# zhoujoey/ORB-SLAM3-Mac

Hardware: AMD Instinct MI355X
Metric: ORB extract+match frames/sec (higher is better)
Workload: dtype u8; 1 GPU; vga: synthetic 640x480 batch=1024 per GPU, 8-level pyramid, 1000 feats/frame, ORB extract + Hamming 2-NN match (Frame.cc:1146) + SearchForInitialization (ORBmatcher.cc:710) vs successor frame; pipelines=1, matchers=side by side (two contexts), frames_total=1024

## Files before the change

### orb-slam3-mac_amd/csrc/match_kernels.hip

```cpp
#include "orb_internal.h"
#include "wave_dpp.h"
#include <climits>
#include <cstring>
#include <string>

struct orbhip_ctx;
hipStream_t orbhip_ctx_stream_internal(orbhip_ctx *c);
void orbhip_set_last_error_internal(const char *msg);
int orbhip_ctx_device_internal(orbhip_ctx *c);
int32_t *orbhip_ctx_status_internal(orbhip_ctx *c);

extern "C" int orbhip_descriptor_distance(const uint8_t *a32, const uint8_t *b32)
{
    int dist = 0;
    for (int i = 0; i < 8; i++) {
        uint32_t pa, pb;
        memcpy(&pa, a32 + 4 * i, 4); memcpy(&pb, b32 + 4 * i, 4);
        uint32_t v = pa ^ pb;
        v = v - ((v >> 1) & 0x55555555);
        v = (v & 0x33333333) + ((v >> 2) & 0x33333333);
        dist += (((v + (v >> 4)) & 0xF0F0F0F) * 0x1010101) >> 24;
    }
    return dist;
}

__device__ __forceinline__ int hamming256(const uint4 &a0, const uint4 &a1, const uint4 &b0, const uint4 &b1)
{
    return __popc(a0.x ^ b0.x) + __popc(a0.y ^ b0.y) + __popc(a0.z ^ b0.z) + __popc(a0.w ^ b0.w) +
           __popc(a1.x ^ b1.x) + __popc(a1.y ^ b1.y) + __popc(a1.z ^ b1.z) + __popc(a1.w ^ b1.w);
}

__device__ __forceinline__ int wave_incl_scan_i(int v) { return wave_scan_add_dpp(v); }

#define BF_TILE 256
__device__ __forceinline__ bool bf_slice(const int32_t *nA, const int32_t *nB, const int32_t *monoA, const int32_t *monoB, int pair, int max_n,
                                         int &na, int &nb, int &ma, int &mb)
{
    na = nA[pair]; nb = nB[pair]; ma = 0; mb = 0;
    if (!monoA) return true;
    if (na > max_n || nb > max_n) return false;
    ma = min(max(monoA[pair], 0), max(na, 0)); mb = min(max(monoB[pair], 0), max(nb, 0));
    na -= ma; nb -= mb;
    return true;
}
template <bool MONO>
__global__ __launch_bounds__(256) void k_bf2nn(const uint8_t *descA, const int32_t *nA, size_t strideA,
                                               const uint8_t *descB, const int32_t *nB, size_t strideB,
                                               int max_n, double ratio, int32_t *idx2, int32_t *dist2, uint8_t *accept,
                                               const int32_t *monoA, const int32_t *monoB)
{
    __shared__ uint4 tile[BF_TILE * 2];
    const int pair = blockIdx.y, tid = threadIdx.x;
    int na, nb, ma, mb;
    if (!bf_slice(nA, nB, MONO ? monoA : nullptr, monoB, pair, max_n, na, nb, ma, mb)) return;
    const int q = blockIdx.x * 256 + tid;
    if (blockIdx.x * 256 >= na) return;
    const uint4 *A = reinterpret_cast<const uint4 *>(descA + (size_t)pair * strideA) + 2 * (size_t)ma;
    const uint4 *B = reinterpret_cast<const uint4 *>(descB + (size_t)pair * strideB) + 2 * (size_t)mb;
    uint4 a0 = make_uint4(0, 0, 0, 0), a1 = a0;
    if (q < na) { a0 = A[2 * q]; a1 = A[2 * q + 1]; }
    uint32_t kb = 0xFFFFFFFFu, ks = 0xFFFFFFFFu;
    for (int t0 = 0; t0 < nb; t0 += BF_TILE) {
        const int tn = min(BF_TILE, nb - t0);
        __syncthreads();
        for (int i = tid; i < tn * 2; i += 256) tile[i] = B[2 * t0 + i];
        __syncthreads();
#pragma unroll 4
        for (int j = 0; j < tn; j++) {
            const uint32_t key = ((uint32_t)hamming256(a0, a1, tile[2 * j], tile[2 * j + 1]) << 16) | (uint32_t)(t0 + j);
            ks = min(ks, max(kb, key));
            kb = min(kb, key);
        }
    }
    if (q < na) {
        const int best = kb == 0xFFFFFFFFu ? INT_MAX : (int)(kb >> 16), second = ks == 0xFFFFFFFFu ? INT_MAX : (int)(ks >> 16);
        const int bi = kb == 0xFFFFFFFFu ? -1 : (int)(kb & 0xFFFFu), si = ks == 0xFFFFFFFFu ? -1 : (int)(ks & 0xFFFFu);
        const size_t o = ((size_t)pair * max_n + q) * 2;
        idx2[o] = bi; idx2[o + 1] = si; dist2[o] = best; dist2[o + 1] = second;
        accept[(size_t)pair * max_n + q] = (si >= 0 && (double)(float)best < (double)(float)second * ratio) ? 1 : 0;
    }
}

#define BFM_ROWB 272
typedef int bfm_v4i __attribute__((ext_vector_type(4)));
typedef int bfm_v16i __attribute__((ext_vector_type(16)));
__device__ __forceinline__ uint32_t bfm_widen4(uint32_t nib) { return __umul24(nib, 0x00204081u) & 0x01010101u; }
__device__ __forceinline__ uint32_t bfm_widen4_pm(uint32_t nib)
{
    uint32_t v = 0;
#pragma unroll
    for (int k = 0; k < 4; k++) v |= (((nib >> k) & 1u) ? 0xFFu : 0x01u) << (8 * k);
    return v;
}
#define BFM_WAVES 8
template <bool MONO>
__global__ __launch_bounds__(64 * BFM_WAVES) void k_bf2nn_mfma(const uint8_t *descA, const int32_t *nA, size_t strideA,
                                                    const uint8_t *descB, const int32_t *nB, size_t strideB,
                                                    int max_n, double ratio, int32_t *idx2, int32_t *dist2, uint8_t *accept,
                                                    const int32_t *monoA, const int32_t *monoB)
{
    __shared__ __attribute__((aligned(16))) uint8_t Bx[2 * 64 * BFM_ROWB];
    static_assert(BFM_WAVES * 2 * 8 * 64 * 4 <= 2 * 64 * BFM_ROWB, "the merge area (half of the rows at a time) fits the tile buffers");
    const int pair = blockIdx.y, tid = threadIdx.x, lane = tid & 63, wave = tid >> 6;
    int na, nb, ma, mb;
    if (!bf_slice(nA, nB, MONO ? monoA : nullptr, monoB, pair, max_n, na, nb, ma, mb)) return;
    const int q0 = blockIdx.x * (32 * BFM_WAVES);
    if (q0 >= na) return;
    const uint32_t *A = reinterpret_cast<const uint32_t *>(descA + (size_t)pair * strideA) + 8 * (size_t)ma;
    const uint32_t *B = reinterpret_cast<const uint32_t *>(descB + (size_t)pair * strideB) + 8 * (size_t)mb;
    const int r = lane & 31, h = lane >> 5;
    const int qrow = q0 + 32 * wave + r;
    bfm_v4i af[8];
    int pa_row = 0;
    {
        uint32_t w[8];
#pragma unroll
        for (int m = 0; m < 8; m++) { w[m] = qrow < na ? A[(size_t)8 * qrow + m] : 0u; pa_row += __popc(w[m]); }
#pragma unroll
        for (int m = 0; m < 8; m++) {
            const uint32_t hw = (w[m] >> (16 * h)) & 0xFFFFu;
            af[m] = (bfm_v4i){(int)bfm_widen4_pm(hw & 15u), (int)bfm_widen4_pm((hw >> 4) & 15u), (int)bfm_widen4_pm((hw >> 8) & 15u), (int)bfm_widen4_pm(hw >> 12)};
        }
    }
    bfm_v16i cinit;
#pragma unroll
    for (int g = 0; g < 16; g++) cinit[g] = __shfl(pa_row, (g & 3) + 8 * (g >> 2) + 4 * h, 64);
    uint32_t k1[16], k2[16];
#pragma unroll
    for (int g = 0; g < 16; g++) { k1[g] = 0xFFFFFFFFu; k2[g] = 0xFFFFFFFFu; }
    const int sc = tid >> 3, sm = tid & 7;
    auto fetch = [&](int t0, uint32_t &w0) { w0 = (t0 + sc < nb) ? B[(size_t)8 * (t0 + sc) + sm] : 0u; };
    auto widen = [&](int bufi, uint32_t w) {
        uint4 lo = make_uint4(bfm_widen4(w & 15u), bfm_widen4((w >> 4) & 15u), bfm_widen4((w >> 8) & 15u), bfm_widen4((w >> 12) & 15u));
        uint4 hi = make_uint4(bfm_widen4((w >> 16) & 15u), bfm_widen4((w >> 20) & 15u), bfm_widen4((w >> 24) & 15u), bfm_widen4(w >> 28));
        uint4 *dst = reinterpret_cast<uint4 *>(&Bx[bufi * 64 * BFM_ROWB + sc * BFM_ROWB + sm * 32]);
        dst[0] = lo; dst[1] = hi;
    };
    uint32_t nw0;
    fetch(0, nw0);
    widen(0, nw0);
    __syncthreads();
    int buf = 0;
    for (int t0 = 0; t0 < nb; t0 += 64, buf ^= 1) {
        const bool more = t0 + 64 < nb;
        if (more) fetch(t0 + 64, nw0);
#pragma unroll
        for (int half = 0; half < 2; half++) {
            if (t0 + 32 * half >= nb) break;
            bfm_v16i acc = cinit;
#pragma unroll
            for (int m = 0; m < 8; m++) {
                const bfm_v4i bf = *reinterpret_cast<const bfm_v4i *>(&Bx[buf * 64 * BFM_ROWB + (r + 32 * half) * BFM_ROWB + m * 32 + h * 16]);
                acc = __builtin_amdgcn_mfma_i32_32x32x32_i8(af[m], bf, acc, 0, 0, 0);
            }
            const int col = t0 + 32 * half + r;
            const uint32_t base = col < nb ? (uint32_t)col : (0x40000000u | (uint32_t)col);
#pragma unroll
            for (int g = 0; g < 16; g++) {
                const uint32_t key = ((uint32_t)acc[g] << 16) + base;
                asm("v_med3_u32 %0, %1, %2, %3" : "=v"(k2[g]) : "v"(k1[g]), "v"(key), "v"(k2[g]));
                k1[g] = min(k1[g], key);
            }
        }
        if (more) widen(buf ^ 1, nw0);
        __syncthreads();
    }
    uint32_t (*kout)[2][8][64] = reinterpret_cast<uint32_t (*)[2][8][64]>(&Bx[0]);
#pragma unroll
    for (int part = 0; part < 2; part++) {
        if (part) __syncthreads();
#pragma unroll
        for (int g = 0; g < 8; g++) { kout[wave][0][g][lane] = k1[8 * part + g]; kout[wave][1][g][lane] = k2[8 * part + g]; }
        __syncthreads();
        if (lane < 16) {
            const int row = 16 * part + lane, g = (row & 3) + 4 * ((row >> 3) & 1), hh = (row >> 2) & 1;
            uint32_t kb = 0xFFFFFFFFu, ks = 0xFFFFFFFFu;
            for (int c = 0; c < 32; c++) {
                const uint32_t a1 = kout[wave][0][g][32 * hh + c], a2 = kout[wave][1][g][32 * hh + c];
                ks = min(min(ks, a2), max(kb, a1));
                kb = min(kb, a1);
            }
            const int q = q0 + 32 * wave + row;
            if (q < na) {
                const bool hb = (kb >> 16) <= 256u, hs = (ks >> 16) <= 256u;
                const int best = hb ? (int)(kb >> 16) : INT_MAX, second = hs ? (int)(ks >> 16) : INT_MAX;
                const int bi = hb ? (int)(kb & 0xFFFFu) : -1, si = hs ? (int)(ks & 0xFFFFu) : -1;
                const size_t o = ((size_t)pair * max_n + q) * 2;
                idx2[o] = bi; idx2[o + 1] = si; dist2[o] = best; dist2[o + 1] = second;
                accept[(size_t)pair * max_n + q] = (si >= 0 && (double)(float)best < (double)(float)second * ratio) ? 1 : 0;
            }
        }
    }
}

extern "C" int orbhip_match_bf2nn_device(orbhip_ctx *ctx, const uint8_t *d_descA, const int32_t *d_nA, size_t strideA,
                                         const uint8_t *d_descB, const int32_t *d_nB, size_t strideB, int pairs,
                                         int max_n, double ratio, int32_t *d_idx2, int32_t *d_dist2, uint8_t *d_accept)
{
    if (!ctx || !d_descA || !d_descB || !d_nA || !d_nB || pairs <= 0 || max_n <= 0 || max_n > 65535 || !d_idx2 || !d_dist2 || !d_accept)
        return ORBHIP_E_BADARG;
    if (hipSetDevice(orbhip_ctx_device_internal(ctx)) != hipSuccess) return ORBHIP_E_HIP;
    if (max_n >= 64 && !getenv("ORBHIP_BF2NN_VALU")) {
        dim3 grid((max_n + 32 * BFM_WAVES - 1) / (32 * BFM_WAVES), pairs);
        hipLaunchKernelGGL(k_bf2nn_mfma<false>, grid, dim3(64 * BFM_WAVES), 0, orbhip_ctx_stream_internal(ctx), d_descA, d_nA, strideA, d_descB, d_nB,
                           strideB, max_n, ratio, d_idx2, d_dist2, d_accept, nullptr, nullptr);
    } else {
        dim3 grid((max_n + 255) / 256, pairs);
        hipLaunchKernelGGL(k_bf2nn<false>, grid, dim3(256), 0, orbhip_ctx_stream_internal(ctx), d_descA, d_nA, strideA, d_descB, d_nB,
                           strideB, max_n, ratio, d_idx2, d_dist2, d_accept, nullptr, nullptr);
    }
    return hipGetLastError() == hipSuccess ? ORBHIP_OK : ORBHIP_E_HIP;
}

int orbhip_bf2nn_slices_internal(orbhip_ctx *ctx, const uint8_t *d_descA, const int32_t *d_nA, const int32_t *d_monoA, size_t strideA,
                                 const uint8_t *d_descB, const int32_t *d_nB, const int32_t *d_monoB, size_t strideB, int pairs, int max_n,
                                 double ratio, int32_t *d_idx2, int32_t *d_dist2, uint8_t *d_accept)
{
    if (max_n >= 64 && !getenv("ORBHIP_BF2NN_VALU")) {
        dim3 grid((max_n + 32 * BFM_WAVES - 1) / (32 * BFM_WAVES), pairs);
        hipLaunchKernelGGL(k_bf2nn_mfma<true>, grid, dim3(64 * BFM_WAVES), 0, orbhip_ctx_stream_internal(ctx), d_descA, d_nA, strideA, d_descB, d_nB,
                           strideB, max_n, ratio, d_idx2, d_dist2, d_accept, d_monoA, d_monoB);
    } else {
        dim3 grid((max_n + 255) / 256, pairs);
        hipLaunchKernelGGL(k_bf2nn<true>, grid, dim3(256), 0, orbhip_ctx_stream_internal(ctx), d_descA, d_nA, strideA, d_descB, d_nB,
                           strideB, max_n, ratio, d_idx2, d_dist2, d_accept, d_monoA, d_monoB);
    }
    return hipGetLastError() == hipSuccess ? ORBHIP_OK : ORBHIP_E_HIP;
}

#define SI_COLS 64
#define SI_ROWS 48
#define SI_MAXN 8192
#define SI_CAP0 4096
#define SI_RANKS 2048
#define SI_TH_LOW 50
#define SI_HISTO 30

template <int NS>
__device__ __forceinline__ int si_register_loop(int lane, int n0, int na0, const float *kx, const float *ky, const uint16_t *cellx, const uint16_t *celly,
                                                const uint16_t *cpos, const uint16_t *gidx, const uint16_t *aidx, uint16_t *bm,
                                                const uint4 *dA, const uint4 *dB, const float *prev, int32_t *m12,
                                                float min_x, float min_y, float inv_w, float inv_h, float r, float nn_ratio)
{
    int nmatches = 0;
    float fkx[NS], fky[NS]; uint32_t fpk[NS]; int fgi[NS], fmd[NS], fm21[NS]; uint4 fd0[NS], fd1[NS];
#pragma unroll
    for (int sl = 0; sl < NS; sl++) {
        const int li = sl * 64 + lane;
        const bool v = li < n0;
        const int lj = v ? li : 0;
        fkx[sl] = kx[lj]; fky[sl] = ky[lj];
        fpk[sl] = v ? ((uint32_t)cellx[lj] | ((uint32_t)celly[lj] << 8) | ((uint32_t)min((int)cpos[lj], SI_RANKS - 1) << 16)) : 0xFFFFu;
        fgi[sl] = v ? (int)gidx[lj] : 0; fmd[sl] = INT_MAX; fm21[sl] = -1;
        fd0[sl] = dB[2 * fgi[sl]]; fd1[sl] = dB[2 * fgi[sl] + 1];
    }
    int qi[NS]; float qx[NS], qy[NS]; uint4 qd0[NS], qd1[NS];
#pragma unroll
    for (int sl = 0; sl < NS; sl++) {
        const int tq = sl * 64 + lane;
        qi[sl] = tq < na0 ? (int)aidx[tq] : 0;
        qx[sl] = prev[2 * qi[sl]]; qy[sl] = prev[2 * qi[sl] + 1];
        qd0[sl] = dA[2 * qi[sl]]; qd1[sl] = dA[2 * qi[sl] + 1];
    }
    for (int t = 0; t < na0; t++) {
        const int tsl = t >> 6, tln = t & 63;
        int i1 = 0; float x = 0, y = 0; uint4 a0 = make_uint4(0, 0, 0, 0), a1 = a0;
#define SI_RL(v) (uint32_t)__builtin_amdgcn_readlane((int)(v), tln)
#pragma unroll
        for (int sl = 0; sl < NS; sl++)
            if (tsl == sl) {
                i1 = (int)SI_RL(qi[sl]); x = __uint_as_float(SI_RL(__float_as_uint(qx[sl]))); y = __uint_as_float(SI_RL(__float_as_uint(qy[sl])));
                a0 = make_uint4(SI_RL(qd0[sl].x), SI_RL(qd0[sl].y), SI_RL(qd0[sl].z), SI_RL(qd0[sl].w));
                a1 = make_uint4(SI_RL(qd1[sl].x), SI_RL(qd1[sl].y), SI_RL(qd1[sl].z), SI_RL(qd1[sl].w));
            }
#undef SI_RL
        int c0 = (int)floorf(__fmul_rn(__fsub_rn(__fsub_rn(x, min_x), r), inv_w)); if (c0 < 0) c0 = 0;
        if (c0 >= SI_COLS) continue;
        int c1 = (int)ceilf(__fmul_rn(__fadd_rn(__fsub_rn(x, min_x), r), inv_w)); if (c1 > SI_COLS - 1) c1 = SI_COLS - 1;
        if (c1 < 0) continue;
        int r0 = (int)floorf(__fmul_rn(__fsub_rn(__fsub_rn(y, min_y), r), inv_h)); if (r0 < 0) r0 = 0;
        if (r0 >= SI_ROWS) continue;
        int r1 = (int)ceilf(__fmul_rn(__fadd_rn(__fsub_rn(y, min_y), r), inv_h)); if (r1 > SI_ROWS - 1) r1 = SI_ROWS - 1;
        if (r1 < 0) continue;
        const int ncy = r1 - r0 + 1;
        uint32_t lk1 = 0xFFFFFFFFu, ld2 = 0xFFFFFFFFu; int best_sl = 0;
        const uint32_t cw = (uint32_t)(c1 - c0), rh = (uint32_t)(r1 - r0);
#pragma unroll
        for (int sl = 0; sl < NS; sl++) {
            if (sl * 64 >= n0) break;
            const uint32_t dcx = (fpk[sl] & 255u) - (uint32_t)c0, dcy = ((fpk[sl] >> 8) & 255u) - (uint32_t)r0;
            const int dist = hamming256(a0, a1, fd0[sl], fd1[sl]);
            const bool c = dcx <= cw && dcy <= rh && fabsf(__fsub_rn(fkx[sl], x)) < r && fabsf(__fsub_rn(fky[sl], y)) < r && !(fmd[sl] <= dist);
            const uint32_t key = c ? ((uint32_t)dist << 23) | ((dcx * (uint32_t)ncy + dcy) * SI_RANKS + (fpk[sl] >> 16)) : 0xFFFFFFFFu;
            ld2 = min(ld2, max(lk1, key));
            best_sl = key < lk1 ? sl : best_sl;
            lk1 = min(lk1, key);
        }
        const uint32_t k1 = wave_min_u32_dpp(lk1);
        const uint32_t k2 = wave_min_u32_dpp(lk1 == k1 ? ld2 : lk1);
        const int d2 = k2 == 0xFFFFFFFFu ? INT_MAX : (int)(k2 >> 23);
        if (k1 == 0xFFFFFFFFu) continue;
        const int best = (int)(k1 >> 23);
        if (!(best <= SI_TH_LOW && (float)best < __fmul_rn((float)d2, nn_ratio))) continue;
        const unsigned long long owner = __ballot(lk1 == k1);
        const int ol = __builtin_amdgcn_readfirstlane(__ffsll((long long)owner) - 1);
        const int bsl = __builtin_amdgcn_readlane(best_sl, ol);
        int old = -1, best_idx = 0;
#pragma unroll
        for (int sl = 0; sl < NS; sl++)
            if (bsl == sl) {
                old = __builtin_amdgcn_readlane(fm21[sl], ol); best_idx = __builtin_amdgcn_readlane(fgi[sl], ol);
                if (lane == ol) { fm21[sl] = i1; fmd[sl] = best; }
            }
        if (old >= 0) nmatches--;
        nmatches++;
        if (lane == 0) {
            if (old >= 0) m12[old] = -1;
            m12[i1] = best_idx;
            bm[i1] = (uint16_t)best_idx;
        }
    }
    return nmatches;
}

__device__ __forceinline__ int si_tail(int lane, int n1, const orbhip_keypoint *kpA, const orbhip_keypoint *kpB, const uint16_t *bm, int8_t *bin_of,
                                       int *hist, int *s_keep, int32_t *m12, float *prev, int nmatches, int check_ori)
{
    const float factor = 1.0f / SI_HISTO;
    __syncthreads();
    if (check_ori) {
        for (int i1 = lane; i1 < n1; i1 += 64) {
            const int b = bm[i1];
            if (b == 0xFFFF) continue;
            float rot = __fsub_rn(kpA[i1].angle, kpB[b].angle);
            if (rot < 0.0f) rot = __fadd_rn(rot, 360.0f);
            int bin = (int)roundf(__fmul_rn(rot, factor));
            if (bin == SI_HISTO) bin = 0;
            atomicAdd(&hist[bin], 1); bin_of[i1] = (int8_t)bin;
        }
        __syncthreads();
        if (lane == 0) {
            int max1 = 0, max2 = 0, max3 = 0, ind1 = -1, ind2 = -1, ind3 = -1;
            for (int i = 0; i < SI_HISTO; i++) {
                const int sz = hist[i];
                if (sz > max1) { max3 = max2; max2 = max1; max1 = sz; ind3 = ind2; ind2 = ind1; ind1 = i; }
                else if (sz > max2) { max3 = max2; max2 = sz; ind3 = ind2; ind2 = i; }
                else if (sz > max3) { max3 = sz; ind3 = i; }
            }
            if ((float)max2 < __fmul_rn(0.1f, (float)max1)) { ind2 = -1; ind3 = -1; }
            else if ((float)max3 < __fmul_rn(0.1f, (float)max1)) ind3 = -1;
            s_keep[0] = ind1; s_keep[1] = ind2; s_keep[2] = ind3;
        }
        __syncthreads();
        int removed = 0;
        for (int i1 = lane; i1 < n1; i1 += 64) {
            const int b = bin_of[i1];
            if (b < 0 || b == s_keep[0] || b == s_keep[1] || b == s_keep[2]) continue;
            if (m12[i1] >= 0) { m12[i1] = -1; removed++; }
        }
        removed = wave_sum_dpp(removed);
        nmatches -= removed;
    }
    __syncthreads();
    for (int i1 = lane; i1 < n1; i1 += 64)
        if (m12[i1] >= 0) { prev[2 * i1] = kpB[m12[i1]].x; prev[2 * i1 + 1] = kpB[m12[i1]].y; }
    return nmatches;
}

#ifdef SI_PROF
__device__ long long g_si_prof[8];
#define SI_T(i) do { if (blockIdx.x == 0 && threadIdx.x == 0) { const long long t_ = clock64(); g_si_prof[i] += t_ - t_prev; t_prev = t_; } } while (0)
extern "C" int orbhip_debug_si_prof(long long *out8, int reset)
{
    if (out8 && hipMemcpyFromSymbol(out8, HIP_SYMBOL(g_si_prof), 64) != hipSuccess) return ORBHIP_E_HIP;
    if (reset) { long long z[8] = {0}; if (hipMemcpyToSymbol(HIP_SYMBOL(g_si_prof), z, 64) != hipSuccess) return ORBHIP_E_HIP; }
    return ORBHIP_OK;
}
#else
#define SI_T(i) do { } while (0)
#endif
__global__ __launch_bounds__(64) void k_search_init(const orbhip_keypoint *kpA_, const uint8_t *descA_, const int32_t *nA,
                                                    const orbhip_keypoint *kpB_, const uint8_t *descB_, const int32_t *nB,
                                                    int max_n, size_t kp_stride, float min_x, float min_y, float max_x, float max_y,
                                                    int window, float nn_ratio, int check_ori, int cap0, int maxn,
                                                    float *prev_, int32_t *m12_, int32_t *nmatches_, int32_t *status, const int32_t *redo_,
                                                    int32_t *redo_out)
{
    if (redo_ && !redo_[blockIdx.x]) { if (redo_out && threadIdx.x == 0) redo_out[blockIdx.x] = 0; return; }
    extern __shared__ __attribute__((aligned(16))) uint8_t si_lds[];
    float *kx = reinterpret_cast<float *>(si_lds), *ky = kx + cap0;
    int *matched_dist = reinterpret_cast<int *>(ky + cap0);
    uint32_t *cand_key = reinterpret_cast<uint32_t *>(matched_dist + cap0);
    uint16_t *cellx = reinterpret_cast<uint16_t *>(cand_key + cap0), *celly = cellx + cap0, *cpos = celly + cap0, *gidx = cpos + cap0;
    int16_t *m21 = reinterpret_cast<int16_t *>(gidx + cap0);
    uint16_t *aidx = reinterpret_cast<uint16_t *>(m21 + cap0), *cand_li = aidx + cap0;
    uint16_t *bm = cand_li + cap0;
    int8_t *bin_of = reinterpret_cast<int8_t *>(bm + maxn);
    __shared__ int hist[SI_HISTO];
    __shared__ int s_keep[3];
    const int pair = blockIdx.x, lane = threadIdx.x;
#ifdef SI_PROF
    long long t_prev = clock64();
#endif
    const unsigned long long lt_mask = (1ull << lane) - 1;
    const int n1 = nA[pair], n2 = nB[pair];
    const orbhip_keypoint *kpA = kpA_ + (size_t)pair * kp_stride, *kpB = kpB_ + (size_t)pair * kp_stride;
    const uint4 *dA = reinterpret_cast<const uint4 *>(descA_ + (size_t)pair * kp_stride * 32);
    const uint4 *dB = reinterpret_cast<const uint4 *>(descB_ + (size_t)pair * kp_stride * 32);
    float *prev = prev_ + (size_t)pair * max_n * 2;
    int32_t *m12 = m12_ + (size_t)pair * max_n;
    if (n1 > maxn || n2 > maxn) { if (lane == 0) { atomicExch(status, ORBHIP_E_CAPACITY); nmatches_[pair] = 0; } return; }
    const float inv_w = __fdiv_rn((float)SI_COLS, __fsub_rn(max_x, min_x));
    const float inv_h = __fdiv_rn((float)SI_ROWS, __fsub_rn(max_y, min_y));
    for (int i = lane; i < SI_HISTO; i += 64) hist[i] = 0;
    int n0 = 0;
    for (int i0 = 0; i0 < n2; i0 += 64) {
        const int i = i0 + lane;
        bool in = false; int px = 0, py = 0; float fx = 0, fy = 0;
        if (i < n2) {
            const orbhip_keypoint k = kpB[i];
            fx = k.x; fy = k.y;
            px = (int)roundf(__fmul_rn(__fsub_rn(fx, min_x), inv_w));
            py = (int)roundf(__fmul_rn(__fsub_rn(fy, min_y), inv_h));
            in = k.octave == 0 && px >= 0 && px < SI_COLS && py >= 0 && py < SI_ROWS;
        }
        const unsigned long long bal = __ballot(in);
        const int li = n0 + __popcll(bal & lt_mask);
        if (in && li < cap0) {
            kx[li] = fx; ky[li] = fy; cellx[li] = (uint16_t)px; celly[li] = (uint16_t)py; gidx[li] = (uint16_t)i;
            matched_dist[li] = INT_MAX; m21[li] = -1;
        }
        n0 += __popcll(bal);
    }
    int na0 = 0;
    for (int i0 = 0; i0 < n1; i0 += 64) {
        const int i = i0 + lane;
        const bool in = i < n1 && kpA[i].octave == 0;
        const unsigned long long bal = __ballot(in);
        const int li = na0 + __popcll(bal & lt_mask);
        if (in && li < cap0) aidx[li] = (uint16_t)i;
        na0 += __popcll(bal);
        if (i < n1) { m12[i] = -1; bin_of[i] = -1; bm[i] = 0xFFFFu; }
    }
    if (redo_out) {
        if (lane == 0) redo_out[pair] = (n0 > cap0 || na0 > cap0) ? 1 : 0;
        if (n0 > cap0 || na0 > cap0) return;
    }
    if (n0 > cap0 || na0 > cap0) { if (lane == 0) { atomicExch(status, ORBHIP_E_CAPACITY); nmatches_[pair] = 0; } return; }
    __syncthreads();
    for (int li = lane; li < n0; li += 64) {
        const int cx = cellx[li], cy = celly[li];
        int rank = 0;
        for (int j = 0; j < li; j++) rank += (cellx[j] == cx && celly[j] == cy);
        cpos[li] = (uint16_t)rank;
    }
    __syncthreads();
    SI_T(0);
    int nmatches = 0;
    const float r = (float)window;
    if (n0 <= 4 * 64 && na0 <= 4 * 64)
        nmatches = si_register_loop<4>(lane, n0, na0, kx, ky, cellx, celly, cpos, gidx, aidx, bm, dA, dB, prev, m12, min_x, min_y, inv_w, inv_h, r, nn_ratio);
    else if (n0 <= 8 * 64 && na0 <= 8 * 64)
        nmatches = si_register_loop<8>(lane, n0, na0, kx, ky, cellx, celly, cpos, gidx, aidx, bm, dA, dB, prev, m12, min_x, min_y, inv_w, inv_h, r, nn_ratio);
    else {
    int i1n = na0 > 0 ? (int)aidx[0] : 0;
    float xn = 0, yn = 0; uint4 pd0 = make_uint4(0, 0, 0, 0), pd1 = pd0;
    if (na0 > 0) { xn = prev[2 * i1n]; yn = prev[2 * i1n + 1]; pd0 = dA[2 * i1n]; pd1 = dA[2 * i1n + 1]; }
    for (int t = 0; t < na0; t++) {
        const int i1 = i1n;
        const float x = xn, y = yn;
        const uint4 a0 = pd0, a1 = pd1;
        if (t + 1 < na0) { i1n = aidx[t + 1]; xn = prev[2 * i1n]; yn = prev[2 * i1n + 1]; pd0 = dA[2 * i1n]; pd1 = dA[2 * i1n + 1]; }
        int c0 = (int)floorf(__fmul_rn(__fsub_rn(__fsub_rn(x, min_x), r), inv_w)); if (c0 < 0) c0 = 0;
        if (c0 >= SI_COLS) continue;
        int c1 = (int)ceilf(__fmul_rn(__fadd_rn(__fsub_rn(x, min_x), r), inv_w)); if (c1 > SI_COLS - 1) c1 = SI_COLS - 1;
        if (c1 < 0) continue;
        int r0 = (int)floorf(__fmul_rn(__fsub_rn(__fsub_rn(y, min_y), r), inv_h)); if (r0 < 0) r0 = 0;
        if (r0 >= SI_ROWS) continue;
        int r1 = (int)ceilf(__fmul_rn(__fadd_rn(__fsub_rn(y, min_y), r), inv_h)); if (r1 > SI_ROWS - 1) r1 = SI_ROWS - 1;
        if (r1 < 0) continue;
        const int ncy = r1 - r0 + 1;
        int ncand = 0;
        for (int l0 = 0; l0 < n0; l0 += 64) {
            const int li = l0 + lane;
            bool c = false; uint32_t key = 0;
            if (li < n0) {
                const int cx = cellx[li], cy = celly[li];
                c = cx >= c0 && cx <= c1 && cy >= r0 && cy <= r1 &&
                    fabsf(__fsub_rn(kx[li], x)) < r && fabsf(__fsub_rn(ky[li], y)) < r;
                key = (uint32_t)(((cx - c0) * ncy + (cy - r0)) * SI_RANKS + min((int)cpos[li], SI_RANKS - 1));
            }
            const unsigned long long bal = __ballot(c);
            if (c) { const int o = ncand + __popcll(bal & lt_mask); cand_li[o] = (uint16_t)li; cand_key[o] = key; }
// ... 1852 lines not shown
```

Before: 317,000 frames/s.

## Software-pipeline MFMA brute-force matcher, interleaving key retirement with next half-tile

Restructures the MFMA Hamming 2-NN loop so the top-2 key updates for one 32-column half-tile are interleaved with the MFMAs of the next half. The accumulator now starts at zero, with the per-row popcount bias applied only once at the end instead of shuffled into an initial accumulator. It also makes the ±1 nibble widening cheaper, adds an occupancy hint to launch_bounds, and spreads the final merge across four lanes per row with xor shuffles instead of serial 32-step loops on 16 lanes. The aim is to hide MFMA latency and cut VALU and merge overhead, at the cost of more complex tail handling and register pressure limits from the occupancy hint.

```diff
diff --git a/orb-slam3-mac_amd/csrc/match_kernels.hip b/orb-slam3-mac_amd/csrc/match_kernels.hip
--- a/orb-slam3-mac_amd/csrc/match_kernels.hip
+++ b/orb-slam3-mac_amd/csrc/match_kernels.hip
@@ -3,6 +3,7 @@
 #include <climits>
 #include <cstring>
 #include <string>
+#include <type_traits>
 
 struct orbhip_ctx;
 hipStream_t orbhip_ctx_stream_internal(orbhip_ctx *c);
@@ -87,14 +88,12 @@
 __device__ __forceinline__ uint32_t bfm_widen4(uint32_t nib) { return __umul24(nib, 0x00204081u) & 0x01010101u; }
 __device__ __forceinline__ uint32_t bfm_widen4_pm(uint32_t nib)
 {
-    uint32_t v = 0;
-#pragma unroll
-    for (int k = 0; k < 4; k++) v |= (((nib >> k) & 1u) ? 0xFFu : 0x01u) << (8 * k);
-    return v;
+    const uint32_t s = bfm_widen4(nib);
+    return ((s << 8) - s) | 0x01010101u;
 }
 #define BFM_WAVES 8
 template <bool MONO>
-__global__ __launch_bounds__(64 * BFM_WAVES) void k_bf2nn_mfma(const uint8_t *descA, const int32_t *nA, size_t strideA,
+__global__ __launch_bounds__(64 * BFM_WAVES, 4) void k_bf2nn_mfma(const uint8_t *descA, const int32_t *nA, size_t strideA,
                                                     const uint8_t *descB, const int32_t *nB, size_t strideB,
                                                     int max_n, double ratio, int32_t *idx2, int32_t *dist2, uint8_t *accept,
                                                     const int32_t *monoA, const int32_t *monoB)
@@ -121,15 +120,13 @@
             const uint32_t hw = (w[m] >> (16 * h)) & 0xFFFFu;
             af[m] = (bfm_v4i){(int)bfm_widen4_pm(hw & 15u), (int)bfm_widen4_pm((hw >> 4) & 15u), (int)bfm_widen4_pm((hw >> 8) & 15u), (int)bfm_widen4_pm(hw >> 12)};
         }
-    }
-    bfm_v16i cinit;
-#pragma unroll
-    for (int g = 0; g < 16; g++) cinit[g] = __shfl(pa_row, (g & 3) + 8 * (g >> 2) + 4 * h, 64);
+        asm volatile("" : "+v"(pa_row));
+    }
     uint32_t k1[16], k2[16];
 #pragma unroll
     for (int g = 0; g < 16; g++) { k1[g] = 0xFFFFFFFFu; k2[g] = 0xFFFFFFFFu; }
     const int sc = tid >> 3, sm = tid & 7;
-    auto fetch = [&](int t0, uint32_t &w0) { w0 = (t0 + sc < nb) ? B[(size_t)8 * (t0 + sc) + sm] : 0u; };
+    auto fetch = [&](int t0, uint32_t &w0) { w0 = (t0 + sc < nb) ? B[(uint32_t)(8 * (t0 + sc) + sm)] : 0u; };
     auto widen = [&](int bufi, uint32_t w) {
         uint4 lo = make_uint4(bfm_widen4(w & 15u), bfm_widen4((w >> 4) & 15u), bfm_widen4((w >> 8) & 15u), bfm_widen4((w >> 12) & 15u));
         uint4 hi = make_uint4(bfm_widen4((w >> 16) & 15u), bfm_widen4((w >> 20) & 15u), bfm_widen4((w >> 24) & 15u), bfm_widen4(w >> 28));
@@ -140,30 +137,76 @@
     fetch(0, nw0);
     widen(0, nw0);
     __syncthreads();
-    int buf = 0;
-    for (int t0 = 0; t0 < nb; t0 += 64, buf ^= 1) {
+    const bfm_v16i zero = {0, 0, 0, 0, 0, 0, 0, 0, 0, 0, 0, 0, 0, 0, 0, 0};
+    bfm_v16i accA = zero, accB = zero;
+    uint32_t baseB = 0;
+    auto retire = [&](const bfm_v16i &acc, uint32_t base, int g) {
+        const uint32_t key = ((uint32_t)acc[g] << 16) + base;
+        asm("v_med3_u32 %1, %0, %2, %1\n\tv_min_u32 %0, %0, %2" : "+v"(k1[g]), "+v"(k2[g]) : "v"(key));
+    };
+    auto key_base = [&](int col) { return (col < nb ? (uint32_t)col : (0x40000000u | (uint32_t)col)) + (256u << 16); };
+    const uint8_t *bx0 = &Bx[r * BFM_ROWB + h * 16];
+    int buf = 0, t0 = 0;
+    auto tile = [&](auto first) {
+        constexpr bool FIRST = decltype(first)::value;
         const bool more = t0 + 64 < nb;
         if (more) fetch(t0 + 64, nw0);
-#pragma unroll
-        for (int half = 0; half < 2; half++) {
-            if (t0 + 32 * half >= nb) break;
-            bfm_v16i acc = cinit;
-#pragma unroll
-            for (int m = 0; m < 8; m++) {
-                const bfm_v4i bf = *reinterpret_cast<const bfm_v4i *>(&Bx[buf * 64 * BFM_ROWB + (r + 32 * half) * BFM_ROWB + m * 32 + h * 16]);
-                acc = __builtin_amdgcn_mfma_i32_32x32x32_i8(af[m], bf, acc, 0, 0, 0);
-            }
-            const int col = t0 + 32 * half + r;
-            const uint32_t base = col < nb ? (uint32_t)col : (0x40000000u | (uint32_t)col);
-#pragma unroll
-            for (int g = 0; g < 16; g++) {
-                const uint32_t key = ((uint32_t)acc[g] << 16) + base;
-                asm("v_med3_u32 %0, %1, %2, %3" : "=v"(k2[g]) : "v"(k1[g]), "v"(key), "v"(k2[g]));
-                k1[g] = min(k1[g], key);
-            }
+        const uint8_t *bx = bx0 + buf * 64 * BFM_ROWB;
+        auto rd = [&](int q) { return *reinterpret_cast<const bfm_v4i *>(bx + (q >> 3) * 32 * BFM_ROWB + (q & 7) * 32); };
+        bfm_v4i bq[4];
+#pragma unroll
+        for (int q = 0; q < 4; q++) bq[q] = rd(q);
+        if constexpr (!FIRST) {
+#pragma unroll
+            for (int g = 0; g < 4; g++) retire(accB, baseB, g);
+        }
+        const uint32_t baseA = key_base(t0 + r);
+#pragma unroll
+        for (int m = 0; m < 8; m++) {
+            accA = __builtin_amdgcn_mfma_i32_32x32x32_i8(af[m], bq[m & 3], m ? accA : zero, 0, 0, 0);
+            bq[m & 3] = rd(m + 4);
+            if constexpr (!FIRST) {
+                retire(accB, baseB, 4 + 3 * (m >> 1) + 2 * (m & 1));
+                if (!(m & 1)) retire(accB, baseB, 5 + 3 * (m >> 1));
+            }
+            __builtin_amdgcn_sched_barrier(0);
+        }
+        baseB = key_base(t0 + 32 + r);
+#pragma unroll
+        for (int m = 0; m < 8; m++) {
+            accB = __builtin_amdgcn_mfma_i32_32x32x32_i8(af[m], bq[m & 3], m ? accB : zero, 0, 0, 0);
+            if (m < 4) bq[m & 3] = rd(m + 12);
+            if (m) {
+                const int g0 = (16 * (m - 1) + 6) / 7, g1 = (16 * m + 6) / 7;
+#pragma unroll
+                for (int g = g0; g < g1; g++) retire(accA, baseA, g);
+            }
+            __builtin_amdgcn_sched_barrier(0);
         }
         if (more) widen(buf ^ 1, nw0);
         __syncthreads();
+        t0 += 64; buf ^= 1;
+    };
+    if (32 < nb) tile(std::true_type());
+    while (t0 + 32 < nb) tile(std::false_type());
+    if (t0 < nb) {
+        const uint8_t *bx = bx0 + buf * 64 * BFM_ROWB;
+        bfm_v4i bq[8];
+#pragma unroll
+        for (int m = 0; m < 8; m++) bq[m] = *reinterpret_cast<const bfm_v4i *>(bx + m * 32);
+#pragma unroll
+        for (int m = 0; m < 8; m++) accA = __builtin_amdgcn_mfma_i32_32x32x32_i8(af[m], bq[m], m ? accA : zero, 0, 0, 0);
+        if (t0) {
+#pragma unroll
+            for (int g = 0; g < 16; g++) retire(accB, baseB, g);
+        }
+        const uint32_t baseA = key_base(t0 + r);
+#pragma unroll
+        for (int g = 0; g < 16; g++) retire(accA, baseA, g);
+        __syncthreads();
+    } else if (nb > 0) {
+#pragma unroll
+        for (int g = 0; g < 16; g++) retire(accB, baseB, g);
     }
     uint32_t (*kout)[2][8][64] = reinterpret_cast<uint32_t (*)[2][8][64]>(&Bx[0]);
 #pragma unroll
@@ -172,23 +215,30 @@
 #pragma unroll
         for (int g = 0; g < 8; g++) { kout[wave][0][g][lane] = k1[8 * part + g]; kout[wave][1][g][lane] = k2[8 * part + g]; }
         __syncthreads();
-        if (lane < 16) {
-            const int row = 16 * part + lane, g = (row & 3) + 4 * ((row >> 3) & 1), hh = (row >> 2) & 1;
-            uint32_t kb = 0xFFFFFFFFu, ks = 0xFFFFFFFFu;
-            for (int c = 0; c < 32; c++) {
-                const uint32_t a1 = kout[wave][0][g][32 * hh + c], a2 = kout[wave][1][g][32 * hh + c];
-                ks = min(min(ks, a2), max(kb, a1));
-                kb = min(kb, a1);
-            }
-            const int q = q0 + 32 * wave + row;
-            if (q < na) {
-                const bool hb = (kb >> 16) <= 256u, hs = (ks >> 16) <= 256u;
-                const int best = hb ? (int)(kb >> 16) : INT_MAX, second = hs ? (int)(ks >> 16) : INT_MAX;
-                const int bi = hb ? (int)(kb & 0xFFFFu) : -1, si = hs ? (int)(ks & 0xFFFFu) : -1;
-                const size_t o = ((size_t)pair * max_n + q) * 2;
-                idx2[o] = bi; idx2[o + 1] = si; dist2[o] = best; dist2[o + 1] = second;
-                accept[(size_t)pair * max_n + q] = (si >= 0 && (double)(float)best < (double)(float)second * ratio) ? 1 : 0;
-            }
+        const int row = 16 * part + (lane >> 2), g = (row & 3) + 4 * ((row >> 3) & 1), hh = (row >> 2) & 1;
+        const int unbias = __shfl(pa_row, row, 64) - 256;
+        uint32_t kb = 0xFFFFFFFFu, ks = 0xFFFFFFFFu;
+#pragma unroll
+        for (int c = 0; c < 8; c++) {
+            const int cc = 32 * hh + 8 * (lane & 3) + ((c + (lane >> 2)) & 7);
+            const uint32_t a1 = kout[wave][0][g][cc], a2 = kout[wave][1][g][cc];
+            ks = min(min(ks, a2), max(kb, a1));
+            kb = min(kb, a1);
+        }
+#pragma unroll
+        for (int s = 1; s < 4; s <<= 1) {
+            const uint32_t pb = __shfl_xor(kb, s, 64), ps = __shfl_xor(ks, s, 64);
+            ks = min(min(ks, ps), max(kb, pb));
+            kb = min(kb, pb);
+        }
+        const int q = q0 + 32 * wave + row;
+        if ((lane & 3) == 0 && q < na) {
+            const bool hb = !(kb & 0x40000000u), hs = !(ks & 0x40000000u);
+            const int best = hb ? (int)(kb >> 16) + unbias : INT_MAX, second = hs ? (int)(ks >> 16) + unbias : INT_MAX;
+            const int bi = hb ? (int)(kb & 0xFFFFu) : -1, si = hs ? (int)(ks & 0xFFFFu) : -1;
+            const size_t o = ((size_t)pair * max_n + q) * 2;
+            idx2[o] = bi; idx2[o + 1] = si; dist2[o] = best; dist2[o + 1] = second;
+            accept[(size_t)pair * max_n + q] = (si >= 0 && (double)(float)best < (double)(float)second * ratio) ? 1 : 0;
         }
     }
 }
```

Result: faster. 321,400 frames/s (median of 6 runs) (+1.4%).
